# NOAA-GFDL/pace

Measured on AMD Instinct MI355X. Metric: simulated-days/day + acoustic-step ms, C768 L79 fp64, 1/2/4/8 MI355X, higher is better.
Workload: dtype f64

## Files before the change

### pace_amd/build.py

```python
from __future__ import annotations

import argparse
import concurrent.futures as cf
import hashlib
import os
import subprocess
import sys

HERE = os.path.dirname(os.path.abspath(__file__))
CSRC = os.path.join(HERE, "csrc")
ROOT = os.path.dirname(HERE)
HOSTEMU_DIR = os.path.join(ROOT, "tests", "_hostemu")

SOURCES = ["fv3_ctx.hip", "fv3_tp2d.hip", "fv3_tp2x.hip", "fv3_tp4.hip", "fv3_tp4x.hip", "fv3_a2b.hip", "fv3_csw.hip", "fv3_dsw.hip", "fv3_wind.hip", "fv3_nh.hip", "fv3_del2x.hip", "fv3_pgf.hip", "fv3_step.hip", "fv3_halo.hip", "fv3_tracer.hip", "fv3_remap.hip"]
HEADERS = ["fv3_common.h", "fv3_ops.h", "fv3_ppm.h", "fv3_a2b.h", "fv3_math.h", "fv3_agpr.h", "fv3_march.h", os.path.join("..", "..", "include", "fv3_mi355x.h")]

HIPCC = os.environ.get("HIPCC", "/opt/rocm/bin/hipcc")
HIP_FLAGS = ["--offload-arch=gfx950", "-std=c++17", "-O3", "-ffp-contract=off", "-fPIC", "-fno-gpu-rdc", "-Wno-unused-result"]
HOST_FLAGS = ["-x", "c++", "-std=c++17", "-O2", "-ffp-contract=off", "-fopenmp", "-fPIC", "-DFV3_HOST_EMU"]


def _tag() -> str:
    t = os.environ.get("FV3_LIB_TAG", "")
    return ("." + t) if t else ""


def lib_path(precision: int = 64, hostemu: bool = False) -> str:
    if hostemu:
        return os.path.join(HOSTEMU_DIR, f"libfv3_hostemu_f{precision}.so")
    return os.path.join(CSRC, f"libfv3_mi355x_f{precision}{_tag()}.so")


def _digest(paths, extra):
    h = hashlib.sha256()
    for p in paths:
        with open(p, "rb") as f:
            h.update(f.read())
    h.update(repr(extra).encode())
    return h.hexdigest()


def src_hash() -> str:
    paths = [os.path.join(CSRC, s) for s in SOURCES] + [os.path.normpath(os.path.join(CSRC, h)) for h in HEADERS]
    return _digest(paths, None)[:16]


def variant_suffix() -> str:
    extra = os.environ.get("FV3_EXTRA_FLAGS", "").split()
# ... 68 lines not shown
```

### pace_amd/csrc/fv3_nh.hip

```cpp
#include "fv3_ops.h"
#include "fv3_math.h"
#include "fv3_agpr.h"

#define K_(arr, k) ((arr) + tb + (long)(k)*g.sk)[pix]

namespace {

struct Sim1 {
  Geo g;
  Real rgas, rgrav, p_fac, ptop;
  template <class Setup, class Finish>
  FV3_HD void run(long tb, unsigned pix, Real dt, const Real *delp, const Real *cappa, const Real *pt, const Real *w1, Real ws, Real *PM, Real *DZ, Real *W2, Real *PP,
                  Real *GAM, Real *PE, Real *wout, Setup setup, Finish finish) const {
    const int nz = g.nz;
    const Real t1g = (Real)2.0 * dt * dt, rdt = (Real)1.0 / dt, r3 = (Real)(1.0 / 3.0);
    auto DM = [&](int k) { return K_(delp, k) * rgrav; };
    auto GM = [&](int k) { return (Real)1.0 / ((Real)1.0 - K_(cappa, k)); };
    {
      Real pm_k, dz_k;
      setup(0, pm_k, dz_k);
      Real dm_m = (Real)0, dm_k = DM(0);
      Real pe_k = fv3_exp(GM(0) * fv3_log(-dm_k / dz_k * rgas * K_(pt, 0))) - pm_k;
      Real bet = (Real)0;
      K_(PP, 0) = (Real)0;
      for (int k = 0; k < nz; ++k) {
        Real bb, dd;
        Real pe_n = (Real)0, dm_n = (Real)0;
        if (k < nz - 1) {
          Real pm_n, dz_n;
          setup(k + 1, pm_n, dz_n);
          dm_n = DM(k + 1);
          const Real g_rat = dm_k / dm_n;
          pe_n = fv3_exp(GM(k + 1) * fv3_log(-dm_n / dz_n * rgas * K_(pt, k + 1))) - pm_n;
          bb = (Real)2.0 * ((Real)1.0 + g_rat);
          dd = (Real)3.0 * (pe_k + g_rat * pe_n);
// ... 124 lines not shown
  }

#ifdef FV3_RIEM_ADDR64
#define KW_(arr, k) ((arr) + tb + (long)(k)*sk)[pix]
#else
#define KW_(arr, k) (*fv3_at((arr) + tb, pix * (unsigned)sizeof(Real) + (unsigned)(k) * (unsigned)(sk * (long)sizeof(Real))))
#endif
#ifndef FV3_RIEM_U
#define FV3_RIEM_U 4
#endif
#ifndef FV3_RIEM_U1
#define FV3_RIEM_U1 8
#endif

#define FV3_KREG_LEVELS (sizeof(Real) == 8 ? FV3_AGPR_LEVELS : FV3_AGPR_LEVELS_F32)
#if defined(__HIP_DEVICE_COMPILE__)
#define KREG_DECL(n)
#define KREG_SET(n, k, v) fv3_agpr_set((k) + 1, (Real)(v))
#define KREG_GET(n, k) fv3_kreg_get((Real)0, (k) + 1)
#define KREG_SET4(n, c, q) fv3_agpr_set4((c) >> 2, (q)[0], (q)[1], (q)[2], (q)[3])
__device__ __attribute__((always_inline)) inline double fv3_kreg_get(double, int k) { return fv3_agpr_get(k); }
__device__ __attribute__((always_inline)) inline float fv3_kreg_get(float, int k) { return fv3_agpr_get_f32(k); }
#else
#define KREG_DECL(n) Real n[FV3_AGPR_LEVELS_F32 + 4]
#define KREG_SET(n, k, v) n[(k) + 1] = (v)
#define KREG_GET(n, k) n[(k) + 1]
#define KREG_SET4(n, c, q) n[c] = (q)[0], n[(c) + 1] = (q)[1], n[(c) + 2] = (q)[2], n[(c) + 3] = (q)[3]
#endif

struct Sim1W {
  long sk;
  int nz;
  Real rgas, rgrav, p_fac, ptop;
  template <bool GL, bool RA, bool ZL = false, class C>
  FV3_HD void run(Real *A, Real *B, long tb, unsigned pix, Real dt, const Real *delp, const Real *cappa, const Real *pt, const Real *qcon, const Real *zint, const Real *w1,
                  Real ws, Real *PM, Real *GAM, Real *wout, C &cl, Real z0 = (Real)0) const {
    const Real t1g = (Real)2.0 * dt * dt, rdt = (Real)1.0 / dt, r3 = (Real)(1.0 / 3.0);
    constexpr int U = FV3_RIEM_U, U1 = FV3_RIEM_U1;
    constexpr int UB = RA ? 1 : U1;
    Real pp_nz;
    KREG_DECL(rg);
#ifdef FV3_RIEM_NO_G4
    constexpr bool G4 = false;
#else
    constexpr bool G4 = RA && U == 4;
#endif
    Real gq[4] = {(Real)0, (Real)0, (Real)0, (Real)0};
    (void)gq;
#define GAM_PUT(k, v)                       \
  do {                                      \
    if constexpr (RA) KREG_SET(rg, k, v);   \
    else if (GL) B[(k)*FV3_WAVE] = (v);     \
    else KW_(GAM, k) = (v);                 \
  } while (0)
#define GAM_PUT_U(k, v)                     \
  do {                                      \
    if constexpr (G4) gq[u_ & 3] = (v);     \
    else GAM_PUT(k, v);                     \
  } while (0)
#define GAM_FLUSH4()                        \
  do {                                      \
    if constexpr (G4) {                     \
      KREG_SET4(rg, c_, gq);                \
      gq[0] = gq[1] = gq[2] = gq[3] = (Real)0; \
    }                                       \
  } while (0)
    {
      Real g_prev = (Real)0, dm_k = (Real)0, pe_k = (Real)0, bet = (Real)0, pp_k = (Real)0;
      Real z_top = ZL ? z0 : KW_(zint, 0);
      auto ld = [&](int k) {
        KRec<5> q;
        q.v[0] = KW_(delp, k);
        q.v[1] = KW_(cappa, k);
        q.v[2] = KW_(pt, k);
        q.v[3] = KW_(qcon, k);
        q.v[4] = ZL ? (Real)0 : KW_(zint, k + 1);
        return q;
      };
      KWALK_E(5, U, true, ld, GAM_FLUSH4(), {
        const int m = K;
        const Real pm_n = cl.pm(m, r.v[0], r.v[3]);
        KW_(PM, m) = pm_n;
        const Real z_lo = ZL ? A[m * FV3_WAVE] : r.v[4];
        const Real dz_n = z_lo - z_top;
        z_top = z_lo;
        const Real dm_n = r.v[0] * rgrav;
        const Real pe_n = fv3_exp(fv3_div((Real)1.0, (Real)1.0 - r.v[1]) * fv3_log(fv3_div(-dm_n, dz_n) * rgas * r.v[2])) - pm_n;
        if (m >= 1) {
          const int k = m - 1;
          const Real g_rat = fv3_div(dm_k, dm_n);
          const Real bb = (Real)2.0 * ((Real)1.0 + g_rat);
          const Real dd = (Real)3.0 * (pe_k + g_rat * pe_n);
          if (k == 0) {
            bet = bb;
            pp_k = fv3_div(dd, bet);
          } else {
            const Real gam = fv3_div(g_prev, bet);
            GAM_PUT_U(k, gam);
            bet = bb - gam;
            pp_k = fv3_div(dd - pp_k, bet);
          }
          A[k * FV3_WAVE] = pp_k;
          g_prev = g_rat;
        }
        dm_k = dm_n;
        pe_k = pe_n;
      })
      {
        const int k = nz - 1;
        const Real bb = (Real)2.0, dd = (Real)3.0 * pe_k;
        const Real gam = fv3_div(g_prev, bet);
        GAM_PUT(k, gam);
        bet = bb - gam;
        pp_k = fv3_div(dd - pp_k, bet);
        A[k * FV3_WAVE] = pp_k;
// ... 70 lines not shown
      KWALK(1, UB, false, ld_gam, {
        if (K >= 1) {
          Real gk;
          if constexpr (RA) gk = KREG_GET(rg, K); else gk = GL ? B[K * FV3_WAVE] : r.v[0];
          const Real wv = A[(K - 1) * FV3_WAVE] - gk * w2_next;
          A[(K - 1) * FV3_WAVE] = wv;
          w2_next = wv;
        }
      })
    }
    {
      Real pe_run = (Real)0;
      auto ld = [&](int k) {
        KRec<2> q;
        q.v[0] = KW_(delp, k);
        q.v[1] = KW_(w1, k);
        return q;
      };
      KWALK(2, U1, true, ld, {
        const Real w2k = A[K * FV3_WAVE];
        pe_run = pe_run + r.v[0] * rgrav * (w2k - r.v[1]) * rdt;
        A[K * FV3_WAVE] = pe_run;
        if (wout) FV3_ST_NT(KW_(wout, K), w2k);
        cl.out_pe(K + 1, pe_run, r.v[0]);
      })
    }
    {
      Real p1 = (Real)0, dm_below = (Real)0, pe1 = A[(nz - 1) * FV3_WAVE], pe2 = (Real)0;
      auto ld = [&](int k) {
        KRec<4> q;
        q.v[0] = KW_(delp, k);
        q.v[1] = KW_(pt, k);
        q.v[2] = KW_(cappa, k);
        q.v[3] = KW_(PM, k);
        return q;
      };
      KWALK(4, U, false, ld, {
        const Real dm = r.v[0] * rgrav;
        const Real pe_k = K >= 1 ? A[(K - 1) * FV3_WAVE] : (Real)0;
        if (K == nz - 1) {
          p1 = (pe_k + (Real)2.0 * pe1) * r3;
        } else {
          const Real g_rat = fv3_div(dm, dm_below);
          const Real bb = (Real)2.0 * ((Real)1.0 + g_rat);
          p1 = (pe_k + bb * pe1 + g_rat * pe2) * r3 - g_rat * p1;
        }
        const Real pmk = r.v[3];
        const Real dzn = -dm * rgas * r.v[1] * fv3_exp((r.v[2] - (Real)1.0) * fv3_log(fv3_max(p_fac * pmk, p1 + pmk)));
        cl.finish(K, dzn);
        pe2 = pe1;
        pe1 = pe_k;
        dm_below = dm;
      })
    }
#undef GAM_PUT
#undef GAM_PUT_U
#undef GAM_FLUSH4
  }
};

#ifndef FV3_RIEM_GL
#define FV3_RIEM_GL 0
#endif
inline bool riem_wave_ok(const Geo &g, bool heavy = false) {
  static const char *e = getenv("FV3_RIEM_MODE");
  if (e && !strcmp(e, "columns")) return false;
  const size_t line = (size_t)g.nz * FV3_WAVE * sizeof(Real) * (FV3_RIEM_GL ? 2 : 1);
  if (heavy && !(e && !strcmp(e, "wave")) && line > 40 * 1024) return false;
  if ((g.nz + 2) * g.sk * (long)sizeof(Real) >= (1L << 32)) return false;
  return line <= (FV3_RIEM_GL ? 160 : 64) * 1024 && g.nz >= 3;
}
inline bool riem_gam_lds(const Geo &) { return FV3_RIEM_GL != 0; }
inline bool riem_reg_arrays(const Geo &g) {
  static const bool off = getenv("FV3_RIEM_REGS") && getenv("FV3_RIEM_REGS")[0] == '0';
  return !off && !FV3_RIEM_GL && g.nz < (int)FV3_KREG_LEVELS;
}

#ifndef PG_KC
#define PG_KC 16
#endif

struct DzcW {
  Real top_ratio, bot_ratio;
};

}

extern "C" int fv3_update_dz_c(fv3_ctx *c, const fv3_field *zs_, const fv3_field *ut_, const fv3_field *vt_, const fv3_field *gz_, const fv3_field *ws_,
                               double dtd, void *stream) {
  return fv3_update_dz_c_from(c, zs_, ut_, vt_, gz_, gz_, ws_, dtd, stream);
}

int fv3_update_dz_c_from(fv3_ctx *c, const fv3_field *zs_, const fv3_field *ut_, const fv3_field *vt_, const fv3_field *gzin_, const fv3_field *gz_,
                         const fv3_field *ws_, double dtd, void *stream) {
  if (!c) return FV3_ERR_ARG;
  FV3_FIELD2D(zs, zs_) FV3_FIELD(ut, ut_) FV3_FIELD(vt, vt_) FV3_FIELD(gz, gz_) FV3_FIELD(gzin, gzin_) FV3_FIELD2D(ws, ws_)
  const Geo g = c->g;
  fv3_stream_t s = (fv3_stream_t)stream;
  const Real dt = (Real)dtd;
  const int nz = g.nz;
  const Real dz_min = (Real)c->cst.dz_min;
  const std::vector<double> &dp = c->dp_ref_h;
  const Real top_ratio = (Real)(dp[0] / (dp[0] + dp[1]));
  const Real bot_ratio = (Real)(dp[nz - 1] / (dp[nz - 2] + dp[nz - 1]));
  Real *gzn = c->scratch[SC_A];
  if (gzin != gz && nz >= 3) {
    launch2(c, s, Box{0, g.nx + 1, 0, g.ny + 1, 0, 0}, [=] FV3_HD(int t, int i, int j) {
      const int fl = g.flags[t];
      const long tb = t * g.st, m2 = t * g.st2;
      const unsigned pix = IX(i, j), qx1 = IX(i + 1, j), qy1 = IX(i, j + 1);
      const unsigned gw = f4_index<1>(g, fl, i - 1, j), gc1 = f4_index<1>(g, fl, i, j), ge = f4_index<1>(g, fl, i + 1, j);
      const unsigned gs = f4_index<2>(g, fl, i, j - 1), gc2 = f4_index<2>(g, fl, i, j), gn = f4_index<2>(g, fl, i, j + 1);
      const Real ar = (g.area + m2)[pix];
// ... 103 lines not shown
    }
  });
  return fv3_post(c, s, "update_dz_c");
}

extern "C" int fv3_riem_solver_c(fv3_ctx *c, double dt2d, const fv3_field *cappa_, double ptopd, const fv3_field *phis_, const fv3_field *ws_,
                                 const fv3_field *ptc_, const fv3_field *q_con_, const fv3_field *delpc_, const fv3_field *gz_, const fv3_field *pef_,
                                 const fv3_field *w3_, void *stream) {
  if (!c) return FV3_ERR_ARG;
  FV3_FIELD(cappa, cappa_) FV3_FIELD2D(phis, phis_) FV3_FIELD2D(ws, ws_) FV3_FIELD(ptc, ptc_) FV3_FIELD(q_con, q_con_) FV3_FIELD(delpc, delpc_)
  FV3_FIELD(gz, gz_) FV3_FIELD(pef, pef_) FV3_FIELD(w3, w3_)
  const Geo g = c->g;
  fv3_stream_t s = (fv3_stream_t)stream;
  const Real dt2 = (Real)dt2d, ptop = (Real)ptopd, grav = (Real)c->cst.grav;
  Sim1 sim{g, (Real)c->cst.rdgas, (Real)1.0 / (Real)c->cst.grav, (Real)c->cfg.p_fac, ptop};
  Real *PM = c->scratch[SC_A], *DZ = c->scratch[SC_B], *W2 = c->scratch[SC_C], *PP = c->scratch[SC_D], *GAM = c->scratch[SC_E];
  const int nz = g.nz;
  if (riem_wave_ok(g)) {
    const Sim1W sw{g.sk, nz, sim.rgas, sim.rgrav, sim.p_fac, ptop};
    const int i0 = 0, j0 = 0, ni = g.nx + 2, ncol = ni * (g.ny + 2);
    const long st = g.st, st2 = g.st2, sk = g.sk;
    const int sj32 = g.sj32, go = g.o;
    const bool gl = riem_gam_lds(g);
    auto go_ = [&](auto ra_tag) {
    constexpr bool RA = decltype(ra_tag)::value;
    launch_waves<1>(c, s, (ncol + FV3_WAVE - 1) / FV3_WAVE, 1, g.nsub, sizeof(Real) * nz * FV3_WAVE * (gl ? 2 : 1), [=] FV3_HD(const Blk &blk, char *smem_) {
      const int t = blk.bz;
      const long tb = t * st;
      FV3_LANES(blk, lane, l) {
        const int cidx = blk.bx * FV3_WAVE + lane;
        if (cidx >= ncol) continue;
        const int jr = cidx / ni;
        const unsigned pix = (unsigned)((j0 + jr + go) * sj32 + (i0 + cidx - jr * ni) + go);
        struct Cl {
          long tb, sk;
          unsigned pix;
          Real peg, pem, z, grav;
          Real *pef, *gz;
          FV3_HD Real pm(int, Real dm, Real qc) {
            const Real peg_n = peg + dm * ((Real)1.0 - qc);
            const Real v = fv3_div(peg_n - peg, fv3_log(fv3_div(peg_n, peg)));
            peg = peg_n;
            return v;
          }
          FV3_HD void out_pe(int k1, Real pe, Real dm) {
            pem = pem + dm;
            FV3_ST_NT(KW_(pef, k1), pe + pem);
          }
          FV3_HD void finish(int k, Real dz) {
            z = z - dz * grav;
            FV3_ST_NT(KW_(gz, k), z);
          }
        };
        const Real z_bot = phis[t * st2 + pix];
        Cl cl{tb, sk, pix, ptop, ptop, z_bot, grav, pef, gz};
        KW_(pef, 0) = ptop;
        sw.run<FV3_RIEM_GL != 0, RA>((Real *)smem_ + lane, (Real *)smem_ + nz * FV3_WAVE + lane, tb, pix, dt2, delpc, cappa, ptc, q_con, gz, w3, ws[t * st2 + pix], PM, GAM, (Real *)nullptr, cl);
        KW_(gz, nz) = z_bot;
      }
    });
    };
    if (riem_reg_arrays(g))
      go_(std::true_type{});
    else
      go_(std::false_type{});
    return fv3_post(c, s, "riem_solver_c");
  }
  launch2(c, s, Box{0, g.nx + 1, 0, g.ny + 1, 0, 0}, [=] FV3_HD(int t, int i, int j) {
    const long tb = t * g.st;
    const unsigned pix = IX(i, j);
    const long p = tb + pix;
    (void)p;
    Real peg = ptop;
    auto setup = [&](int k, Real &pm, Real &dz) {
      const Real dm = K_(delpc, k);
      const Real peg_n = peg + dm * ((Real)1.0 - K_(q_con, k));
      pm = (peg_n - peg) / fv3_log(peg_n / peg);
      dz = K_(gz, k + 1) - K_(gz, k);
      K_(PM, k) = pm;
      K_(DZ, k) = dz;
      peg = peg_n;
    };
    Real z = phis[t * g.st2 + IX(i, j)];
    const Real z_bot = z;
    auto finish = [&](int k, Real dz) {
      z = z - dz * grav;
      K_(gz, k) = z;
    };
    sim.run(tb, pix, dt2, delpc, cappa, ptc, w3, ws[t * g.st2 + IX(i, j)], PM, DZ, W2, PP, GAM, pef, (Real *)nullptr, setup, finish);
    K_(gz, nz) = z_bot;
    Real pem = ptop;
    K_(pef, 0) = ptop;
    for (int k = 0; k < nz; ++k) {
      pem = pem + K_(delpc, k);
      K_(pef, k + 1) = K_(pef, k + 1) + pem;
    }
  });
  return fv3_post(c, s, "riem_solver_c");
}

extern "C" int fv3_riem_solver3(fv3_ctx *c, int last_call, double dtd, const fv3_field *cappa_, double ptopd, const fv3_field *zs_, const fv3_field *wsd_,
                                const fv3_field *delz_, const fv3_field *q_con_, const fv3_field *delp_, const fv3_field *pt_, const fv3_field *zh_,
                                const fv3_field *pe_, const fv3_field *ppe_, const fv3_field *pk3_, const fv3_field *pk_, const fv3_field *peln_,
                                const fv3_field *w_, void *stream) {
  if (!c) return FV3_ERR_ARG;
  FV3_FIELD(cappa, cappa_) FV3_FIELD2D(zs, zs_) FV3_FIELD2D(wsd, wsd_) FV3_FIELD(delz, delz_) FV3_FIELD(q_con, q_con_) FV3_FIELD(delp, delp_)
  FV3_FIELD(pt, pt_) FV3_FIELD(zh, zh_) FV3_FIELD(pe, pe_) FV3_FIELD(ppe, ppe_) FV3_FIELD(pk3, pk3_) FV3_FIELD(pk, pk_) FV3_FIELD(peln, peln_)
  FV3_FIELD(w, w_)
  const Geo g = c->g;
  fv3_stream_t s = (fv3_stream_t)stream;
  const Real dt = (Real)dtd, ptop = (Real)ptopd;
  const Real akap = (Real)(c->cst.rdgas / c->cst.cp_air);
  Sim1 sim{g, (Real)c->cst.rdgas, (Real)1.0 / (Real)c->cst.grav, (Real)c->cfg.p_fac, ptop};
  Real *PM = c->scratch[SC_A], *W2 = c->scratch[SC_C], *PP = c->scratch[SC_D], *GAM = c->scratch[SC_E];
  const int nz = g.nz;
  const bool last = last_call != 0;
  if (riem_wave_ok(g, true)) {
    const Sim1W sw{g.sk, nz, sim.rgas, sim.rgrav, sim.p_fac, ptop};
    const int i0 = 1, j0 = 1, ni = g.nx, ncol = ni * g.ny;
    const long st = g.st, st2 = g.st2, sk = g.sk;
    const int sj32 = g.sj32, go = g.o;
    const bool gl = riem_gam_lds(g);
    const ColumnOrder ord{g.nx, g.ny, c->frame_pass != 0 ? FV3_FRAME_W : 0};
    const int nwave = (ncol + FV3_WAVE - 1) / FV3_WAVE;
    const int nwave_frame = c->frame_pass != 0 ? (ord.n_frame() + FV3_WAVE - 1) / FV3_WAVE : 0;
    const int w_lo = c->frame_pass == 2 ? nwave_frame : 0, w_hi = c->frame_pass == 1 ? nwave_frame : nwave;
    Real *const zn = c->dz_scan_src;
    const char *sde = getenv("FV3_SEQ_DELZ");
    const bool store_delz = !(c->seq_delz_dead && !(sde && !strcmp(sde, "every")));
    const bool pre = zn != nullptr;
    const Real dzm = c->dz_scan_min;
// ... 866 lines not shown
```

### pace_amd/csrc/fv3_ops.h

```cpp
#pragma once
#include "fv3_common.h"

enum {
  SC_TP_FY2 = 0,
  SC_TP_FX2 = 1,
  SC_TP_QI = 2,
  SC_TP_QJ = 3,
  SC_DN_D2 = 4,
  SC_DN_FX = 5,
  SC_DN_FY = 6,
  SC_A = 7,
  SC_B = 8,
  SC_C = 9,
  SC_D = 10,
  SC_E = 11,
  SC_F = 12,
  SC_G = 13,
  SC_H = 14,
  SC_I = 15,
  SC_J = 16,
  SC_K = 17,
  SC_L = 18,
  SC_M = 19,
  SC_N = 20,
// ... 88 lines not shown
  Real dt, dddmp;
  int hord;
  bool store_dn;
  int k0, k1;
  Real *u_side = nullptr, *v_side = nullptr;
  int side_seg = 0;
};
void wind_stage_march(fv3_ctx *c, fv3_stream_t s, const WindStage &a);
int sx_march_seg(const fv3_ctx *c, int nk);

void tracer_pair_stream(fv3_ctx *c, fv3_stream_t s, const DswScalars &a);

#ifndef FV3_Q4_KB_DEFAULT
#define FV3_Q4_KB_DEFAULT 16
#endif
void del6_vt_flux_edge_strips(fv3_ctx *c, fv3_stream_t s, const Real *q, Real *d2, Real *fx2, Real *fy2, const Deln &dn, bool q_raw, int k0, int k1);
void del6_vt_flux_patches(fv3_ctx *c, fv3_stream_t s, const Real *q, Real *d2, Real *fx2, Real *fy2, const Deln &dn, bool q_raw, int k0, int k1);
void del6_vt_flux(fv3_ctx *c, fv3_stream_t s, const Real *q, Real *d2, Real *fx2, Real *fy2, const Deln &dn, bool q_raw, int k0, int k1);

void a2b_ord4(fv3_ctx *c, fv3_stream_t s, Real *qin, Real *qout, int kin0, int kout0, int nk, bool replace, Real scale = (Real)1);
int fv3_d_sw_out(fv3_ctx *c, const fv3_field *delpc, const fv3_field *delp, const fv3_field *pt, const fv3_field *u, const fv3_field *v, const fv3_field *w,
                 const fv3_field *uc, const fv3_field *vc, const fv3_field *ua, const fv3_field *va, const fv3_field *divgd, const fv3_field *mfx,
                 const fv3_field *mfy, const fv3_field *cx, const fv3_field *cy, const fv3_field *crx, const fv3_field *cry, const fv3_field *xfx,
                 const fv3_field *yfx, const fv3_field *q_con, const fv3_field *zh, const fv3_field *heat_source, const fv3_field *diss_est, double dt,
                 void *stream, const fv3_field *o_delp, const fv3_field *o_pt, const fv3_field *o_w, const fv3_field *o_q_con, int (*after_scalars)(void *) = nullptr,
                 void *after_user = nullptr);
int fv3_csw_join(fv3_ctx *c, void *stream);
void nh_pgf_fused(fv3_ctx *c, fv3_stream_t s, const Real *pp, const Real *pk3, const Real *gz, const Real *delp, Real *u, Real *v, Real dt, Real top, Real gz_scale,
                  int pass);
int fv3_nh_p_grad_scaled(fv3_ctx *c, const fv3_field *u, const fv3_field *v, const fv3_field *pp, const fv3_field *gz, const fv3_field *pk3, const fv3_field *delp,
                         double dt, double ptop, double akap, double gz_scale, void *stream);
int fv3_update_dz_c_from(fv3_ctx *c, const fv3_field *zs, const fv3_field *ut, const fv3_field *vt, const fv3_field *gz_in, const fv3_field *gz, const fv3_field *ws,
                         double dt, void *stream);
```

### pace_amd/csrc/fv3_step.hip

```cpp
#include <chrono>

#include "fv3_ops.h"

namespace {

struct OpTimer {
  fv3_ctx *c;
  fv3_stream_t s;
  int id;
  bool on;
#ifdef FV3_HOST_EMU
  std::chrono::steady_clock::time_point t0;
#else
  hipEvent_t e0, e1;
#endif
  OpTimer(fv3_ctx *c_, fv3_stream_t s_, int id_)
      : c(c_), s(s_), id(id_), on(c_->profiling == 1 || (c_->profiling == 2 && (id_ == FV3_OP_D_SW || c_->prof_parent == FV3_OP_D_SW))) {
    if (!on) return;
#ifdef FV3_HOST_EMU
    t0 = std::chrono::steady_clock::now();
#else
    (void)hipEventCreate(&e0);
    (void)hipEventCreate(&e1);
    (void)hipEventRecord(e0, s);
// ... 229 lines not shown
      c->seq_delz_dead = false;
      c->seq_uava_thin = false;
      c->seq_acc_defer = false;
      c->seq_acc_sum_n = 0;
      c->dz_scan_src = nullptr;
    }
  } pp_guard{c, stream};

  if (pingpong) {
    const fv3_field *fs[4] = {&st->delp, &st->pt, &st->w, &st->q_con}, *fd[4] = {&f_delp[1], &f_pt[1], &f_w[1], &f_qc[1]};
    RUN(FV3_OP_GLUE, copy_frames(c, 4, fs, fd, stream));
  }
  HALO(FV3_HALO_Q_CON__CAPPA, 0);
  HALO(FV3_HALO_DELP__PT, 0);
  HALO(FV3_HALO_U__V, 0);
  HALO(FV3_HALO_Q_CON__CAPPA, 1);
  (void)n_map;
  const char *acc_env = getenv("FV3_ACC_STORE");
  const bool acc_store = !(acc_env && acc_env[0] == '0') && n_split > 0 && dsw_honors_acc_first(c);
  if (!acc_store) {
    const fv3_field *acc[4] = {&st->mfxd, &st->mfyd, &st->cxd, &st->cyd};
    for (int a = 0; a < 4; ++a) RUN(FV3_OP_GLUE, fv3_zero(c, acc[a], stream));
  }
  const bool heat_reset = n_map == 1 || !fv3_alt("heat_zero_first_call");
  const bool heat_store = acc_store && heat_reset && cf.d_con > 1.0e-5 && !fv3_alt("heat_zero_first_call");
  if (heat_reset && !heat_store) RUN(FV3_OP_GLUE, fv3_zero(c, &ws->heat_source, stream));
  const bool acc_defer = acc_store && n_split >= 2 && n_split <= FV3_ACC_MAXSTEPS && dsw_can_defer_acc(c) && fv3_acc_slots_ensure(c, n_split);
  if (getenv("FV3_DEBUG_FD")) fprintf(stderr, "[acoustic_step] accumulators: %s\n", acc_defer ? "cx / cy formed once per call from the sub-steps' Courant numbers, mfx / mfy read-modify-write" : acc_store ? "read-modify-write, first sub-step stores" : "zeroed, read-modify-write");
  if (acc_store)
    RUN(FV3_OP_GLUE, zero_unwritten(c, &st->mfxd, &st->mfyd, &st->cxd, &st->cyd, heat_store ? &ws->heat_source : nullptr, stream));
  RUN(FV3_OP_GLUE, fv3_zero(c, &st->diss_estd, stream));
  const char *gz_env = getenv("FV3_GZ_FIRST");
  const bool gz_direct = !(gz_env && !strcmp(gz_env, "copy"));
  for (int it = 0; it < n_split; ++it) {
    const int remap_step = it == n_split - 1;
    if (!w_started) HALO(FV3_HALO_W, 0);
    w_started = false;
    if (it == 0) {
      RUN(FV3_OP_GLUE, fv3_set_gz(c, &ws->zs, &st->delz, gz_direct ? &ws->zh : &ws->gz, stream));
      HALO(gz_direct ? FV3_HALO_ZH : FV3_HALO_GZ, 0);
      HALO(FV3_HALO_DELP__PT, 1);
    }
    HALO(FV3_HALO_U__V, 1);
    HALO(FV3_HALO_W, 1);
    c->seq_csw_defer = (gz_direct || it > 0) && c->g.nz >= 3;
    c->seq_uava_thin = it < n_split - 1;
    RUN(FV3_OP_C_SW, fv3_c_sw(c, &f_delp[cur], &f_pt[cur], &st->u, &st->v, &f_w[cur], &st->uc, &st->vc, &st->ua, &st->va, &ws->ut, &ws->vt, &ws->divgd, &st->omga,
                              &ws->delpc, &ws->ptc, dt2, stream));
    c->seq_csw_defer = false;
    c->seq_uava_thin = false;
    if (cf.nord > 0) HALO(FV3_HALO_DIVGD, 0);
    if (it == 0 && gz_direct) {
      HALO(FV3_HALO_ZH, 1);
      RUN(FV3_OP_UPDATE_DZ_C, fv3_update_dz_c_from(c, &ws->zs, &ws->ut, &ws->vt, &ws->zh, &ws->gz, &ws->ws3, dt2, stream));
    } else if (it == 0) {
      HALO(FV3_HALO_GZ, 1);
      RUN(FV3_OP_GLUE, fv3_copy(c, &ws->gz, &ws->zh, stream));
      RUN(FV3_OP_UPDATE_DZ_C, fv3_update_dz_c(c, &ws->zs, &ws->ut, &ws->vt, &ws->gz, &ws->ws3, dt2, stream));
    } else {
      RUN(FV3_OP_UPDATE_DZ_C, fv3_update_dz_c_from(c, &ws->zs, &ws->ut, &ws->vt, &ws->zh, &ws->gz, &ws->ws3, dt2, stream));
    }
    RUN(FV3_OP_GLUE, fv3_csw_join(c, stream));
    RUN(FV3_OP_RIEM_SOLVER_C,
        fv3_riem_solver_c(c, dt2, &st->cappa, ptop, &st->phis, &ws->ws3, &ws->ptc, &f_qc[cur], &ws->delpc, &ws->gz, &ws->pkc, &st->omga, stream));
    if (frame_first) {
      c->frame_pass = 1;
      RUN(FV3_OP_P_GRAD_C, fv3_p_grad_c(c, &st->uc, &st->vc, &ws->delpc, &ws->pkc, &ws->gz, dt2, stream));
      HALO(FV3_HALO_UC__VC, 0);
      c->frame_pass = 2;
      RUN(FV3_OP_P_GRAD_C, fv3_p_grad_c(c, &st->uc, &st->vc, &ws->delpc, &ws->pkc, &ws->gz, dt2, stream));
      c->frame_pass = 0;
    } else {
      RUN(FV3_OP_P_GRAD_C, fv3_p_grad_c(c, &st->uc, &st->vc, &ws->delpc, &ws->pkc, &ws->gz, dt2, stream));
      HALO(FV3_HALO_UC__VC, 0);
    }
    if (cf.nord > 0) HALO(FV3_HALO_DIVGD, 1);
    HALO(FV3_HALO_UC__VC, 1);
    fv3_field f_crx = ws->crx, f_cry = ws->cry;
    if (acc_defer) {
      f_crx.ptr = c->acc_slots[2 * it];
      f_cry.ptr = c->acc_slots[2 * it + 1];
      c->seq_acc_defer = true;
      c->seq_acc_sum_n = it == n_split - 1 ? n_split : 0;
    }
    if (pingpong) {
      const int nxt = 1 - cur;
      struct Mid {
        fv3_ctx *c;
        int pp_n_next;
        void *stream;
        fv3_stream_t s;
      } mid{c, nxt ? 4 : 0, stream, s};
      auto start_halo = [](void *u) -> int {
        Mid *m = (Mid *)u;
        fv3_ctx *c = m->c;
        fv3_stream_t s = m->s;
        m->c->pp_n = m->pp_n_next;
// ... 118 lines not shown
```

Before: 210.3.

## Keep riem_solver_c PM column in high AGPRs and add column-wise dz_c kernels

Adds an AGPR-backed store (a160-a255) that holds the first 48 levels of the PM column in the C-grid Riemann solver, so those values are not written to and re-read from global scratch. Adds new column kernels: one for update_dz_c, and one for riem_solver_c that can optionally fuse the dz_c sweep as a pre-sweep through LDS. By default the acoustic step now runs the separate column dz_c kernel followed by the PM-in-registers solver. The fused path is opt-in through an environment variable. The change trades global memory traffic for register-file pressure and jump-table asm overhead, and the clobbered AGPRs may lower occupancy.

```diff
diff --git a/pace_amd/build.py b/pace_amd/build.py
--- a/pace_amd/build.py
+++ b/pace_amd/build.py
@@ -13,7 +13,7 @@
 HOSTEMU_DIR = os.path.join(ROOT, "tests", "_hostemu")
 
 SOURCES = ["fv3_ctx.hip", "fv3_tp2d.hip", "fv3_tp2x.hip", "fv3_tp4.hip", "fv3_tp4x.hip", "fv3_a2b.hip", "fv3_csw.hip", "fv3_dsw.hip", "fv3_wind.hip", "fv3_nh.hip", "fv3_del2x.hip", "fv3_pgf.hip", "fv3_step.hip", "fv3_halo.hip", "fv3_tracer.hip", "fv3_remap.hip"]
-HEADERS = ["fv3_common.h", "fv3_ops.h", "fv3_ppm.h", "fv3_a2b.h", "fv3_math.h", "fv3_agpr.h", "fv3_march.h", os.path.join("..", "..", "include", "fv3_mi355x.h")]
+HEADERS = ["fv3_common.h", "fv3_ops.h", "fv3_ppm.h", "fv3_a2b.h", "fv3_math.h", "fv3_agpr.h", "fv3_agpr_hi.h", "fv3_march.h", os.path.join("..", "..", "include", "fv3_mi355x.h")]
 
 HIPCC = os.environ.get("HIPCC", "/opt/rocm/bin/hipcc")
 HIP_FLAGS = ["--offload-arch=gfx950", "-std=c++17", "-O3", "-ffp-contract=off", "-fPIC", "-fno-gpu-rdc", "-Wno-unused-result"]
diff --git a/pace_amd/csrc/fv3_agpr_hi.h b/pace_amd/csrc/fv3_agpr_hi.h
--- /dev/null
+++ b/pace_amd/csrc/fv3_agpr_hi.h
@@ -0,0 +1,25 @@
+#pragma once
+#include "fv3_agpr.h"
+
+#define FV3_AGPR_HI_LEVELS 48
+#if defined(__HIP_DEVICE_COMPILE__)
+#define FV3_AGH_CASES(X) \
+ X(160, 161) X(162, 163) X(164, 165) X(166, 167) X(168, 169) X(170, 171) X(172, 173) X(174, 175) \
+  X(176, 177) X(178, 179) X(180, 181) X(182, 183) X(184, 185) X(186, 187) X(188, 189) X(190, 191) \
+  X(192, 193) X(194, 195) X(196, 197) X(198, 199) X(200, 201) X(202, 203) X(204, 205) X(206, 207) \
+  X(208, 209) X(210, 211) X(212, 213) X(214, 215) X(216, 217) X(218, 219) X(220, 221) X(222, 223) \
+  X(224, 225) X(226, 227) X(228, 229) X(230, 231) X(232, 233) X(234, 235) X(236, 237) X(238, 239) \
+  X(240, 241) X(242, 243) X(244, 245) X(246, 247) X(248, 249) X(250, 251) X(252, 253) X(254, 255)
+#define FV3_AGH_CLOBBERS "a160", "a161", "a162", "a163", "a164", "a165", "a166", "a167", "a168", "a169", "a170", "a171", "a172", "a173", "a174", "a175", "a176", "a177", "a178", "a179", "a180", "a181", "a182", "a183", "a184", "a185", "a186", "a187", "a188", "a189", "a190", "a191", "a192", "a193", "a194", "a195", "a196", "a197", "a198", "a199", "a200", "a201", "a202", "a203", "a204", "a205", "a206", "a207", "a208", "a209", "a210", "a211", "a212", "a213", "a214", "a215", "a216", "a217", "a218", "a219", "a220", "a221", "a222", "a223", "a224", "a225", "a226", "a227", "a228", "a229", "a230", "a231", "a232", "a233", "a234", "a235", "a236", "a237", "a238", "a239", "a240", "a241", "a242", "a243", "a244", "a245", "a246", "a247", "a248", "a249", "a250", "a251", "a252", "a253", "a254", "a255"
+__device__ __attribute__((always_inline)) inline void fv3_agpr_hi_set(int k, double v) {
+  const int lo = __double2loint(v), hi = __double2hiint(v);
+  const int t = k * 20 + 12;
+  asm volatile(FV3_AG_JUMP FV3_AGH_CASES(FV3_AG_W) ".LFV3AG%=:\n" : : [t] "s"(t), [lo] "v"(lo), [hi] "v"(hi) : "vcc", "scc", FV3_AGH_CLOBBERS);
+}
+__device__ __attribute__((always_inline)) inline double fv3_agpr_hi_get(int k) {
+  int lo, hi;
+  const int t = k * 20 + 12;
+  asm volatile(FV3_AG_JUMP FV3_AGH_CASES(FV3_AG_R) ".LFV3AG%=:\n" : [lo] "=&v"(lo), [hi] "=&v"(hi) : [t] "s"(t) : "vcc", "scc", FV3_AGH_CLOBBERS);
+  return __hiloint2double(hi, lo);
+}
+#endif
diff --git a/pace_amd/csrc/fv3_nh.hip b/pace_amd/csrc/fv3_nh.hip
--- a/pace_amd/csrc/fv3_nh.hip
+++ b/pace_amd/csrc/fv3_nh.hip
@@ -1,6 +1,7 @@
 #include "fv3_ops.h"
 #include "fv3_math.h"
 #include "fv3_agpr.h"
+#include "fv3_agpr_hi.h"
 
 #define K_(arr, k) ((arr) + tb + (long)(k)*g.sk)[pix]
 
@@ -191,7 +192,7 @@
   long sk;
   int nz;
   Real rgas, rgrav, p_fac, ptop;
-  template <bool GL, bool RA, bool ZL = false, class C>
+  template <bool GL, bool RA, bool ZL = false, bool PMR0 = false, class C>
   FV3_HD void run(Real *A, Real *B, long tb, unsigned pix, Real dt, const Real *delp, const Real *cappa, const Real *pt, const Real *qcon, const Real *zint, const Real *w1,
                   Real ws, Real *PM, Real *GAM, Real *wout, C &cl, Real z0 = (Real)0) const {
     const Real t1g = (Real)2.0 * dt * dt, rdt = (Real)1.0 / dt, r3 = (Real)(1.0 / 3.0);
@@ -199,6 +200,16 @@
     constexpr int UB = RA ? 1 : U1;
     Real pp_nz;
     KREG_DECL(rg);
+    constexpr bool PMR = PMR0 && RA && sizeof(Real) == 8;
+#if defined(__HIP_DEVICE_COMPILE__)
+#define PMH_SET(k, v) fv3_agpr_hi_set(k, (double)(v))
+#define PMH_GET(k) (Real) fv3_agpr_hi_get(k)
+#else
+    Real pmh[FV3_AGPR_HI_LEVELS];
+    (void)pmh;
+#define PMH_SET(k, v) pmh[k] = (v)
+#define PMH_GET(k) pmh[k]
+#endif
 #ifdef FV3_RIEM_NO_G4
     constexpr bool G4 = false;
 #else
@@ -239,7 +250,14 @@
       KWALK_E(5, U, true, ld, GAM_FLUSH4(), {
         const int m = K;
         const Real pm_n = cl.pm(m, r.v[0], r.v[3]);
-        KW_(PM, m) = pm_n;
+        if constexpr (PMR) {
+          if (m < FV3_AGPR_HI_LEVELS)
+            PMH_SET(m, pm_n);
+          else
+            KW_(PM, m) = pm_n;
+        } else {
+          KW_(PM, m) = pm_n;
+        }
         const Real z_lo = ZL ? A[m * FV3_WAVE] : r.v[4];
         const Real dz_n = z_lo - z_top;
         z_top = z_lo;
@@ -376,7 +394,7 @@
         q.v[0] = KW_(delp, k);
         q.v[1] = KW_(pt, k);
         q.v[2] = KW_(cappa, k);
-        q.v[3] = KW_(PM, k);
+        q.v[3] = PMR && k < FV3_AGPR_HI_LEVELS ? (Real)0 : KW_(PM, k);
         return q;
       };
       KWALK(4, U, false, ld, {
@@ -389,7 +407,10 @@
           const Real bb = (Real)2.0 * ((Real)1.0 + g_rat);
           p1 = (pe_k + bb * pe1 + g_rat * pe2) * r3 - g_rat * p1;
         }
-        const Real pmk = r.v[3];
+        Real pmk = r.v[3];
+        if constexpr (PMR) {
+          if (K < FV3_AGPR_HI_LEVELS) pmk = PMH_GET(K);
+        }
         const Real dzn = -dm * rgas * r.v[1] * fv3_exp((r.v[2] - (Real)1.0) * fv3_log(fv3_max(p_fac * pmk, p1 + pmk)));
         cl.finish(K, dzn);
         pe2 = pe1;
@@ -397,6 +418,8 @@
         dm_below = dm;
       })
     }
+#undef PMH_SET
+#undef PMH_GET
 #undef GAM_PUT
 #undef GAM_PUT_U
 #undef GAM_FLUSH4
@@ -423,6 +446,27 @@
 #ifndef PG_KC
 #define PG_KC 16
 #endif
+
+struct RiemCCl {
+  long tb, sk;
+  unsigned pix;
+  Real peg, pem, z, grav;
+  Real *pef, *gz;
+  FV3_HD Real pm(int, Real dm, Real qc) {
+    const Real peg_n = peg + dm * ((Real)1.0 - qc);
+    const Real v = fv3_div(peg_n - peg, fv3_log(fv3_div(peg_n, peg)));
+    peg = peg_n;
+    return v;
+  }
+  FV3_HD void out_pe(int k1, Real pe, Real dm) {
+    pem = pem + dm;
+    FV3_ST_NT(KW_(pef, k1), pe + pem);
+  }
+  FV3_HD void finish(int k, Real dz) {
+    z = z - dz * grav;
+    FV3_ST_NT(KW_(gz, k), z);
+  }
+};
 
 struct DzcW {
   Real top_ratio, bot_ratio;
@@ -592,28 +636,8 @@
         if (cidx >= ncol) continue;
         const int jr = cidx / ni;
         const unsigned pix = (unsigned)((j0 + jr + go) * sj32 + (i0 + cidx - jr * ni) + go);
-        struct Cl {
-          long tb, sk;
-          unsigned pix;
-          Real peg, pem, z, grav;
-          Real *pef, *gz;
-          FV3_HD Real pm(int, Real dm, Real qc) {
-            const Real peg_n = peg + dm * ((Real)1.0 - qc);
-            const Real v = fv3_div(peg_n - peg, fv3_log(fv3_div(peg_n, peg)));
-            peg = peg_n;
-            return v;
-          }
-          FV3_HD void out_pe(int k1, Real pe, Real dm) {
-            pem = pem + dm;
-            FV3_ST_NT(KW_(pef, k1), pe + pem);
-          }
-          FV3_HD void finish(int k, Real dz) {
-            z = z - dz * grav;
-            FV3_ST_NT(KW_(gz, k), z);
-          }
-        };
         const Real z_bot = phis[t * st2 + pix];
-        Cl cl{tb, sk, pix, ptop, ptop, z_bot, grav, pef, gz};
+        RiemCCl cl{tb, sk, pix, ptop, ptop, z_bot, grav, pef, gz};
         KW_(pef, 0) = ptop;
         sw.run<FV3_RIEM_GL != 0, RA>((Real *)smem_ + lane, (Real *)smem_ + nz * FV3_WAVE + lane, tb, pix, dt2, delpc, cappa, ptc, q_con, gz, w3, ws[t * st2 + pix], PM, GAM, (Real *)nullptr, cl);
         KW_(gz, nz) = z_bot;
@@ -657,6 +681,192 @@
     }
   });
   return fv3_post(c, s, "riem_solver_c");
+}
+
+namespace {
+template <bool LDS, int UF>
+FV3_HD inline void dzc_column(const Geo &g, int t, int i, int j, int c0, int ni, const Real *ut, const Real *vt, const Real *zh, const Real *zs, Real *gz,
+                              Real top_ratio, Real bot_ratio, Real dz_min, Real dt2, Real *A_, Real &ws_v, Real &z0) {
+  const int nz = g.nz;
+  const long tb = t * g.st, sk = g.sk;
+  const int fl = g.flags[t];
+  const unsigned pix = IX(i, j), qx1 = IX(i + 1, j), qy1 = IX(i, j + 1);
+  const unsigned gw = f4_index<1>(g, fl, i - 1, j), gc1 = f4_index<1>(g, fl, i, j), ge = f4_index<1>(g, fl, i + 1, j);
+  const unsigned gs = f4_index<2>(g, fl, i, j - 1), gc2 = f4_index<2>(g, fl, i, j), gn = f4_index<2>(g, fl, i, j + 1);
+  const Real ar = (g.area + t * g.st2)[pix];
+  auto at = [&](const Real *f, unsigned q, int k) -> Real { return *fv3_at(f + tb, q * (unsigned)sizeof(Real) + (unsigned)k * (unsigned)(g.sk * (long)sizeof(Real))); };
+  Real ax0 = at(ut, pix, nz - 1), ax1 = at(ut, qx1, nz - 1), ay0 = at(vt, pix, nz - 1), ay1 = at(vt, qy1, nz - 1);
+  Real cx0 = (Real)0, cx1 = (Real)0, cy0 = (Real)0, cy1 = (Real)0, px0 = (Real)0, px1 = (Real)0, py0 = (Real)0, py1 = (Real)0;
+  Real below = (Real)0;
+  {
+    auto ld = [&](int k, auto full_tag) {
+      constexpr bool FULL = decltype(full_tag)::value;
+      KRec<FULL ? 11 : 9> q;
+      const bool has = k >= 2;
+      q.v[0] = has ? at(ut, pix, k - 2) : (Real)0;
+      q.v[1] = has ? at(ut, qx1, k - 2) : (Real)0;
+      q.v[2] = has ? at(vt, pix, k - 2) : (Real)0;
+      q.v[3] = has ? at(vt, qy1, k - 2) : (Real)0;
+      q.v[4] = at(zh, pix, k);
+      q.v[5] = at(zh, gw, k);
+      q.v[6] = at(zh, ge, k);
+      q.v[7] = at(zh, gs, k);
+      q.v[8] = at(zh, gn, k);
+      if constexpr (FULL) {
+        q.v[9] = at(zh, gc1, k);
+        q.v[10] = at(zh, gc2, k);
+      }
+      return q;
+    };
+    auto ld_full = [&](int k) { return ld(k, std::true_type{}); };
+    auto ld_fast = [&](int k) { return ld(k, std::false_type{}); };
+#define DZC_STEP(ZC1, ZE, ZS, ZC2, ZN) \
+      const int k = K;                                                                                                                            \
+      const Real nx0 = r.v[0], nx1 = r.v[1], ny0 = r.v[2], ny1 = r.v[3], zc = r.v[4], zw = r.v[5], zc1 = ZC1, ze = ZE, zsn = ZS, zc2 = ZC2, zno = ZN;\
+      Real x0, x1, y0, y1;                                                                                                                        \
+      if (k == g.nz) {                                                                                                                            \
+        x0 = ax0 + (ax0 - nx0) * bot_ratio;                                                                                                       \
+        x1 = ax1 + (ax1 - nx1) * bot_ratio;                                                                                                       \
+        y0 = ay0 + (ay0 - ny0) * bot_ratio;                                                                                                       \
+        y1 = ay1 + (ay1 - ny1) * bot_ratio;                                                                                                       \
+      } else if (k == 0) {                                                                                                                        \
+        x0 = cx0 + (cx0 - px0) * top_ratio;                                                                                                       \
+        x1 = cx1 + (cx1 - px1) * top_ratio;                                                                                                       \
+        y0 = cy0 + (cy0 - py0) * top_ratio;                                                                                                       \
+        y1 = cy1 + (cy1 - py1) * top_ratio;                                                                                                       \
+      } else {                                                                                                                                    \
+        const Real d1 = g.dp_ref[k], d0 = g.dp_ref[k - 1];                                                                                        \
+        const Real int_ratio = (Real)1.0 / (d0 + d1);                                                                                             \
+        x0 = (d1 * ax0 + d0 * cx0) * int_ratio;                                                                                                   \
+        x1 = (d1 * ax1 + d0 * cx1) * int_ratio;                                                                                                   \
+        y0 = (d1 * ay0 + d0 * cy0) * int_ratio;                                                                                                   \
+        y1 = (d1 * ay1 + d0 * cy1) * int_ratio;                                                                                                   \
+      }                                                                                                                                           \
+      const Real fx0 = x0 * (x0 > (Real)0 ? zw : zc1);                                                                                            \
+      const Real fx1 = x1 * (x1 > (Real)0 ? zc1 : ze);                                                                                            \
+      const Real fy0 = y0 * (y0 > (Real)0 ? zsn : zc2);                                                                                           \
+      const Real fy1 = y1 * (y1 > (Real)0 ? zc2 : zno);                                                                                           \
+      const Real zn = (zc * ar + fx0 - fx1 + fy0 - fy1) / (ar + x0 - x1 + y0 - y1);                                                               \
+      Real v = zn;                                                                                                                                \
+      if (k == g.nz)                                                                                                                              \
+        ws_v = (zs[t * g.st2 + pix] - zn) / dt2;                                                                                                    \
+      else                                                                                                                                        \
+        v = fv3_max(zn, below + dz_min);                                                                                                          \
+      KW_(gz, k) = v;                                                                                                                             \
+      if constexpr (LDS) {                                                                                                                        \
+        if (k >= 1)                                                                                                                               \
+          A_[(k - 1) * FV3_WAVE] = v;                                                                                                             \
+        else                                                                                                                                      \
+          z0 = v;                                                                                                                                 \
+      }                                                                                                                                           \
+      below = v;                                                                                                                                  \
+      px0 = cx0;                                                                                                                                  \
+      px1 = cx1;                                                                                                                                  \
+      py0 = cy0;                                                                                                                                  \
+      py1 = cy1;                                                                                                                                  \
+      cx0 = ax0;                                                                                                                                  \
+      cx1 = ax1;                                                                                                                                  \
+      cy0 = ay0;                                                                                                                                  \
+      cy1 = ay1;                                                                                                                                  \
+      ax0 = nx0;                                                                                                                                  \
+      ax1 = nx1;                                                                                                                                  \
+      ay0 = ny0;                                                                                                                                  \
+      ay1 = ny1;                                                                                                                                  
+    const int c1 = c0 + FV3_WAVE - 1;
+    auto in_wave = [&](int q) { return q >= c0 && q <= c1; };
+    const bool corner = in_wave(0) || in_wave(ni - 1) || in_wave((g.ny + 1) * ni) || in_wave((g.ny + 1) * ni + ni - 1);
+    const int nz = g.nz + 1;
+    if (corner) {
+      KWALK(11, 2, false, ld_full, { DZC_STEP(r.v[9], r.v[6], r.v[7], r.v[10], r.v[8]) })
+    } else {
+      KWALK(9, UF, false, ld_fast, { DZC_STEP(r.v[4], r.v[6], r.v[7], r.v[4], r.v[8]) })
+    }
+#undef DZC_STEP
+  }
+  (void)A_;
+  (void)z0;
+}
+
+}
+
+bool fv3_csw_columns_ok(const fv3_ctx *c) { return c && c->g.nz >= 3 && riem_wave_ok(c->g) && riem_reg_arrays(c->g) && !riem_gam_lds(c->g); }
+
+int fv3_dzc_columns(fv3_ctx *c, const fv3_field *zs_, const fv3_field *ut_, const fv3_field *vt_, const fv3_field *zh_, const fv3_field *gz_, const fv3_field *ws_,
+                    double dt2d, void *stream) {
+  if (!fv3_csw_columns_ok(c)) return FV3_ERR_ARG;
+  FV3_FIELD2D(zs, zs_) FV3_FIELD2D(ws, ws_) FV3_FIELD(ut, ut_) FV3_FIELD(vt, vt_) FV3_FIELD(zh, zh_) FV3_FIELD(gz, gz_)
+  if (zh == gz) return FV3_ERR_ARG;
+  const Geo g = c->g;
+  fv3_stream_t s = (fv3_stream_t)stream;
+  const Real dt2 = (Real)dt2d, dz_min = (Real)c->cst.dz_min;
+  const int nz = g.nz;
+  const std::vector<double> &dp = c->dp_ref_h;
+  const Real top_ratio = (Real)(dp[0] / (dp[0] + dp[1]));
+  const Real bot_ratio = (Real)(dp[nz - 1] / (dp[nz - 2] + dp[nz - 1]));
+  const int ni = g.nx + 2, ncol = ni * (g.ny + 2);
+  launch_waves<3>(c, s, (ncol + FV3_WAVE - 1) / FV3_WAVE, 1, g.nsub, 0, [=] FV3_HD(const Blk &blk, char *) {
+    const int t = blk.bz;
+    FV3_LANES(blk, lane, l) {
+      const int cidx = blk.bx * FV3_WAVE + lane;
+      if (cidx >= ncol) continue;
+      const int j = cidx / ni, i = cidx - j * ni;
+      Real ws_v = (Real)0, z0 = (Real)0;
+      dzc_column<false, 2>(g, t, i, j, blk.bx * FV3_WAVE, ni, ut, vt, zh, zs, gz, top_ratio, bot_ratio, dz_min, dt2, (Real *)nullptr, ws_v, z0);
+      ws[t * g.st2 + IX(i, j)] = ws_v;
+    }
+  });
+  return fv3_post(c, s, "update_dz_c");
+}
+
+int fv3_csw_columns(fv3_ctx *c, bool presweep, const fv3_field *zs_, const fv3_field *ut_, const fv3_field *vt_, const fv3_field *zh_, const fv3_field *ws_,
+                    const fv3_field *gz_, double dt2d,
+                    const fv3_field *cappa_, double ptopd, const fv3_field *phis_, const fv3_field *ptc_, const fv3_field *q_con_, const fv3_field *delpc_,
+                    const fv3_field *pef_, const fv3_field *w3_, void *stream) {
+  if (!fv3_csw_columns_ok(c)) return FV3_ERR_ARG;
+  FV3_FIELD2D(zs, zs_) FV3_FIELD2D(ws, ws_) FV3_FIELD(ut, ut_) FV3_FIELD(vt, vt_) FV3_FIELD(zh, zh_) FV3_FIELD(gz, gz_) FV3_FIELD(cappa, cappa_) FV3_FIELD2D(phis, phis_)
+  FV3_FIELD(ptc, ptc_) FV3_FIELD(q_con, q_con_) FV3_FIELD(delpc, delpc_) FV3_FIELD(pef, pef_) FV3_FIELD(w3, w3_)
+  if (presweep && zh == gz) return FV3_ERR_ARG;
+  const Geo g = c->g;
+  fv3_stream_t s = (fv3_stream_t)stream;
+  const Real dt2 = (Real)dt2d, ptop = (Real)ptopd, grav = (Real)c->cst.grav;
+  const int nz = g.nz;
+  const Sim1W sw{g.sk, nz, (Real)c->cst.rdgas, (Real)1.0 / (Real)c->cst.grav, (Real)c->cfg.p_fac, ptop};
+  const Real dz_min = (Real)c->cst.dz_min;
+  const std::vector<double> &dp = c->dp_ref_h;
+  const Real top_ratio = (Real)(dp[0] / (dp[0] + dp[1]));
+  const Real bot_ratio = (Real)(dp[nz - 1] / (dp[nz - 2] + dp[nz - 1]));
+  Real *PM = c->scratch[SC_A], *GAM = c->scratch[SC_E];
+  const int ni = g.nx + 2, ncol = ni * (g.ny + 2);
+  const long st = g.st, st2 = g.st2, sk = g.sk;
+  auto go_ = [&](auto pre_tag) {
+  constexpr bool PRE = decltype(pre_tag)::value;
+  launch_waves<1>(c, s, (ncol + FV3_WAVE - 1) / FV3_WAVE, 1, g.nsub, sizeof(Real) * nz * FV3_WAVE, [=] FV3_HD(const Blk &blk, char *smem_) {
+    const int t = blk.bz;
+    const long tb = t * st;
+    FV3_LANES(blk, lane, l) {
+      const int cidx = blk.bx * FV3_WAVE + lane;
+      if (cidx >= ncol) continue;
+      const int j = cidx / ni, i = cidx - j * ni;
+      Real *A_ = (Real *)smem_ + lane;
+      const unsigned pix = IX(i, j);
+      Real ws_v = (Real)0, z0 = (Real)0;
+      if constexpr (!PRE)
+        ws_v = ws[t * st2 + pix];
+      else
+        dzc_column<true, 4>(g, t, i, j, blk.bx * FV3_WAVE, ni, ut, vt, zh, zs, gz, top_ratio, bot_ratio, dz_min, dt2, A_, ws_v, z0);
+      const Real z_bot = phis[t * st2 + pix];
+      RiemCCl cl{tb, sk, pix, ptop, ptop, z_bot, grav, pef, gz};
+      KW_(pef, 0) = ptop;
+      sw.run<false, true, PRE, true>(A_, (Real *)nullptr, tb, pix, dt2, delpc, cappa, ptc, q_con, gz, w3, ws_v, PM, GAM, (Real *)nullptr, cl, z0);
+      KW_(gz, nz) = z_bot;
+    }
+  });
+  };
+  if (presweep)
+    go_(std::true_type{});
+  else
+    go_(std::false_type{});
+  return fv3_post(c, s, "csw_columns");
 }
 
 extern "C" int fv3_riem_solver3(fv3_ctx *c, int last_call, double dtd, const fv3_field *cappa_, double ptopd, const fv3_field *zs_, const fv3_field *wsd_,
diff --git a/pace_amd/csrc/fv3_ops.h b/pace_amd/csrc/fv3_ops.h
--- a/pace_amd/csrc/fv3_ops.h
+++ b/pace_amd/csrc/fv3_ops.h
@@ -144,3 +144,10 @@
                          double dt, double ptop, double akap, double gz_scale, void *stream);
 int fv3_update_dz_c_from(fv3_ctx *c, const fv3_field *zs, const fv3_field *ut, const fv3_field *vt, const fv3_field *gz_in, const fv3_field *gz, const fv3_field *ws,
                          double dt, void *stream);
+
+bool fv3_csw_columns_ok(const fv3_ctx *c);
+int fv3_csw_columns(fv3_ctx *c, bool presweep, const fv3_field *zs, const fv3_field *ut, const fv3_field *vt, const fv3_field *zh, const fv3_field *ws,
+                    const fv3_field *gz, double dt2, const fv3_field *cappa, double ptop, const fv3_field *phis, const fv3_field *ptc, const fv3_field *q_con,
+                    const fv3_field *delpc, const fv3_field *pef, const fv3_field *w3, void *stream);
+int fv3_dzc_columns(fv3_ctx *c, const fv3_field *zs, const fv3_field *ut, const fv3_field *vt, const fv3_field *zh, const fv3_field *gz, const fv3_field *ws,
+                    double dt2, void *stream);
diff --git a/pace_amd/csrc/fv3_step.hip b/pace_amd/csrc/fv3_step.hip
--- a/pace_amd/csrc/fv3_step.hip
+++ b/pace_amd/csrc/fv3_step.hip
@@ -285,6 +285,14 @@
   RUN(FV3_OP_GLUE, fv3_zero(c, &st->diss_estd, stream));
   const char *gz_env = getenv("FV3_GZ_FIRST");
   const bool gz_direct = !(gz_env && !strcmp(gz_env, "copy"));
+  const char *dzc_env = getenv("FV3_DZC_SCAN");
+  const bool dzc_fused = fv3_csw_columns_ok(c) && dzc_env && !strcmp(dzc_env, "presweep");
+  const bool dzc_columns = fv3_csw_columns_ok(c) && !(dzc_env && !strcmp(dzc_env, "separate"));
+  const char *pm_env = getenv("FV3_RIEM_PM");
+  const bool pm_regs = fv3_csw_columns_ok(c) && !(pm_env && !strcmp(pm_env, "memory"));
+  if (getenv("FV3_DEBUG_FD"))
+    fprintf(stderr, "[acoustic_step] update_dz_c: %s; riem_solver_c: %s\n", dzc_fused ? "pre-sweep of riem_solver_c" : "own kernel",
+            dzc_fused || pm_regs ? "PM in registers" : "PM through memory");
   for (int it = 0; it < n_split; ++it) {
     const int remap_step = it == n_split - 1;
     if (!w_started) HALO(FV3_HALO_W, 0);
@@ -303,19 +311,30 @@
     c->seq_csw_defer = false;
     c->seq_uava_thin = false;
     if (cf.nord > 0) HALO(FV3_HALO_DIVGD, 0);
-    if (it == 0 && gz_direct) {
-      HALO(FV3_HALO_ZH, 1);
-      RUN(FV3_OP_UPDATE_DZ_C, fv3_update_dz_c_from(c, &ws->zs, &ws->ut, &ws->vt, &ws->zh, &ws->gz, &ws->ws3, dt2, stream));
-    } else if (it == 0) {
-      HALO(FV3_HALO_GZ, 1);
-      RUN(FV3_OP_GLUE, fv3_copy(c, &ws->gz, &ws->zh, stream));
-      RUN(FV3_OP_UPDATE_DZ_C, fv3_update_dz_c(c, &ws->zs, &ws->ut, &ws->vt, &ws->gz, &ws->ws3, dt2, stream));
-    } else {
-      RUN(FV3_OP_UPDATE_DZ_C, fv3_update_dz_c_from(c, &ws->zs, &ws->ut, &ws->vt, &ws->zh, &ws->gz, &ws->ws3, dt2, stream));
-    }
-    RUN(FV3_OP_GLUE, fv3_csw_join(c, stream));
-    RUN(FV3_OP_RIEM_SOLVER_C,
-        fv3_riem_solver_c(c, dt2, &st->cappa, ptop, &st->phis, &ws->ws3, &ws->ptc, &f_qc[cur], &ws->delpc, &ws->gz, &ws->pkc, &st->omga, stream));
+    if (it == 0 && gz_direct) HALO(FV3_HALO_ZH, 1);
+    if (dzc_fused && (it > 0 || gz_direct)) {
+      RUN(FV3_OP_GLUE, fv3_csw_join(c, stream));
+      RUN(FV3_OP_RIEM_SOLVER_C, fv3_csw_columns(c, true, &ws->zs, &ws->ut, &ws->vt, &ws->zh, &ws->ws3, &ws->gz, dt2, &st->cappa, ptop, &st->phis, &ws->ptc,
+                                                &f_qc[cur], &ws->delpc, &ws->pkc, &st->omga, stream));
+    } else {
+      if ((it == 0 && gz_direct) || it > 0) {
+        if (dzc_columns)
+          RUN(FV3_OP_UPDATE_DZ_C, fv3_dzc_columns(c, &ws->zs, &ws->ut, &ws->vt, &ws->zh, &ws->gz, &ws->ws3, dt2, stream));
+        else
+          RUN(FV3_OP_UPDATE_DZ_C, fv3_update_dz_c_from(c, &ws->zs, &ws->ut, &ws->vt, &ws->zh, &ws->gz, &ws->ws3, dt2, stream));
+      } else {
+        HALO(FV3_HALO_GZ, 1);
+        RUN(FV3_OP_GLUE, fv3_copy(c, &ws->gz, &ws->zh, stream));
+        RUN(FV3_OP_UPDATE_DZ_C, fv3_update_dz_c(c, &ws->zs, &ws->ut, &ws->vt, &ws->gz, &ws->ws3, dt2, stream));
+      }
+      RUN(FV3_OP_GLUE, fv3_csw_join(c, stream));
+      if (pm_regs)
+        RUN(FV3_OP_RIEM_SOLVER_C, fv3_csw_columns(c, false, &ws->zs, &ws->ut, &ws->vt, &ws->zh, &ws->ws3, &ws->gz, dt2, &st->cappa, ptop, &st->phis, &ws->ptc,
+                                                  &f_qc[cur], &ws->delpc, &ws->pkc, &st->omga, stream));
+      else
+        RUN(FV3_OP_RIEM_SOLVER_C,
+            fv3_riem_solver_c(c, dt2, &st->cappa, ptop, &st->phis, &ws->ws3, &ws->ptc, &f_qc[cur], &ws->delpc, &ws->gz, &ws->pkc, &st->omga, stream));
+    }
     if (frame_first) {
       c->frame_pass = 1;
       RUN(FV3_OP_P_GRAD_C, fv3_p_grad_c(c, &st->uc, &st->vc, &ws->delpc, &ws->pkc, &ws->gz, dt2, stream));
```

Result: no change. 210.8, median of 6 (+0.2%).
